# gorgonia/agogo

Measured on AMD Instinct MI355X. Metric: mcts_sims_per_sec, higher is better.
Workload: dtype f32 (Winograd F(5x5,3x3): fp32 transforms; transform-domain products as fp16x2 = each fp32 operand scaled by a power of two and split into 2 fp16 pieces (22-23 significand bits, absolute error <= 2^-38 of the tensor range), 3 fp16 MFMAs per product, fp32 accumulate)

## Files before the change

agogo_amd/csrc/conv_wino_h2.hpp:

```cpp
#pragma once

template <int TM> struct WinoT;
template <> struct WinoT<4> {
  static constexpr int AL = 6, VSHIFT = 7;
  static constexpr float BT[6][6] = {{4, 0, -5, 0, 1, 0}, {0, -4, -4, 1, 1, 0}, {0, 4, -4, -1, 1, 0}, {0, -2, -1, 2, 1, 0}, {0, 2, -1, -2, 1, 0}, {0, 4, 0, -5, 0, 1}};
  static constexpr float AT[4][6] = {{1, 1, 1, 1, 1, 0}, {0, 1, -1, 2, -2, 0}, {0, 1, 1, 4, 4, 0}, {0, 1, -1, 8, -8, 1}};
  static constexpr double G[6][3] = {{1.0 / 4, 0, 0}, {-1.0 / 6, -1.0 / 6, -1.0 / 6}, {-1.0 / 6, 1.0 / 6, -1.0 / 6}, {1.0 / 24, 1.0 / 12, 1.0 / 6}, {1.0 / 24, -1.0 / 12, 1.0 / 6}, {0, 0, 1}};
};
template <> struct WinoT<5> {
  static constexpr int AL = 7, VSHIFT = 6;
  static constexpr float BT[7][7] = {{-0.5f, 0.25f, 2.5f, -1.25f, -2, 1, 0}, {0, 0.5f, 0.25f, -2.25f, -1, 1, 0}, {0, -0.5f, 0.75f, 1.75f, -3, 1, 0},
                                     {0, 1, 1.5f, -2, -1.5f, 1, 0},          {0, -1, 2.5f, 0, -2.5f, 1, 0},       {0, 0.25f, 0, -1.25f, 0, 1, 0},
                                     {0, -0.5f, 0.25f, 2.5f, -1.25f, -2, 1}};
  static constexpr float AT[5][7] = {{1, 1, 1, 1, 1, 1, 0}, {0, 1, -1, 0.5f, -0.5f, 2, 0}, {0, 1, 1, 0.25f, 0.25f, 4, 0}, {0, 1, -1, 0.125f, -0.125f, 8, 0},
                                     {0, 1, 1, 0.0625f, 0.0625f, 16, 1}};
  static constexpr double G[7][3] = {{-2, 0, 0}, {-2.0 / 3, -2.0 / 3, -2.0 / 3}, {-2.0 / 9, 2.0 / 9, -2.0 / 9}, {16.0 / 9, 8.0 / 9, 4.0 / 9}, {16.0 / 15, -8.0 / 15, 4.0 / 15},
                                     {2.0 / 45, 4.0 / 45, 8.0 / 45}, {0, 0, 1}};
};
template <int TM> __device__ __forceinline__ void wino_btv(const float* d, float* o);
template <int TM> __device__ __forceinline__ void wino_atv(const float* m, float* o);
template <> __device__ __forceinline__ void wino_btv<4>(const float* d, float* o) { wino_bt6(d, o); }
template <> __device__ __forceinline__ void wino_atv<4>(const float* m, float* o) { wino_at4(m, o); }
template <> __device__ __forceinline__ void wino_btv<5>(const float* d, float* o) {
  o[0] = -0.5f * d[0] + 0.25f * d[1] + 2.5f * d[2] - 1.25f * d[3] - 2.f * d[4] + d[5];
// ... 33 lines not shown
  float* wave_max;
  float w_unscale;
  const float* t_in;
  const float* col_unscale;
  const float* t_next;
  int cform;
  const _Float16* U2c;
  const float* amax_true;
  const float* wm_prev;
  float* wm_out;
  unsigned* amax_next;
  float g1, g0;
  int gemm_variant;
  int temporal_stores;
  int live_r, live_c;
  int row_pad;
};
__device__ __forceinline__ size_t h2_row(const WinoH2Args& h, int pos, int t) {
  return (size_t)(t >> h.rsh) * h.rA + (size_t)pos * h.rB + (size_t)(t & h.rmask);
}

__device__ __forceinline__ void wino_h2_scales(unsigned amax_bits, int shift, float* s, float* inv) {
  int e = (int)((amax_bits >> 23) & 0xffu);
  if (amax_bits == 0u) { *s = 1.f; *inv = 1.f; return; }
  e = e < 30 ? 30 : (e > 230 ? 230 : e);
  *s = __uint_as_float((unsigned)(268 - shift - e) << 23);
  *inv = __uint_as_float((unsigned)(e - 14 + shift) << 23);
}

__device__ __forceinline__ unsigned wino_h2_pack(float a, float b, unsigned* lo) {
// ... 50 lines not shown
#pragma unroll
    for (int i = 0; i < AL; i++) {
      const bool ok = okx && TM * ty + i < a.Hp;
      dx[i] = ok ? d[i][j].x : 0.f; dy[i] = ok ? d[i][j].y : 0.f;
    }
    wino_btv<TM>(dx, ox);
    wino_btv<TM>(dy, oy);
#pragma unroll
    for (int i = 0; i < AL; i++) { tmx[i][j] = ox[i]; tmy[i][j] = oy[i]; }
  }
  unsigned* V2 = reinterpret_cast<unsigned*>(a.V);
  const int c = 2 * c2;
  const size_t word_in_row = (size_t)(c >> 5) * 32 + ((c & 31) >> 1);
  const int lane = threadIdx.x & 63;
  const size_t swap_word = (size_t)((c2 >> 6) * 4) * 32 + lane;
  const int row_r = (h.cform && h.live_r) ? maps::rows_row(maps::ROWS_R, a.nty, a.ntx, b % (128 / a.TPB), ty, tx) : (t & 127);
  const int row_c = (h.cform && h.live_c) ? maps::rows_row(maps::ROWS_C, a.nty, a.ntx, b % (128 / a.TPB), ty, tx) : (t & 127);
#pragma unroll
  for (int i = 0; i < AL; i++) {
    float ox[AL], oy[AL];
    wino_btv<TM>(tmx[i], ox);
    wino_btv<TM>(tmy[i], oy);
#pragma unroll
    for (int j = 0; j < AL; j++) {
      unsigned lo;
      const unsigned hi = wino_h2_pack(ox[j] * sbx, oy[j] * sby, &lo);
      if (h.cform) {
        const auto s16 = __builtin_amdgcn_permlane16_swap(hi, lo, false, false);
        const unsigned e0 = s16[0], e1 = s16[1];
        const int NS = a.C >> 5;
        const size_t chunk0 = ((size_t)(t >> 7) * h.npos + (size_t)(i * AL + j)) * NS + (size_t)((c2 >> 6) * 4 + 2 * (lane >> 5));
        const int cls = maps::rows_class(true, true, AL, i, j);
        const int row = cls == maps::ROWS_R ? row_r : (cls == maps::ROWS_C ? row_c : (t & 127));
        if (row < 0) continue;
        unsigned* p0 = V2 + chunk0 * 4096 + (size_t)row * 32 + (lane & 31);
        p0[0] = e0;
        p0[4096] = e1;
        continue;
      }
      unsigned* rowp = V2 + h2_row(h, i * AL + j, t) * a.C;
      if (h.in_swap) {
        const auto s16 = __builtin_amdgcn_permlane16_swap(hi, lo, false, false);
        const unsigned e0 = s16[0], e1 = s16[1];
        const auto s32 = __builtin_amdgcn_permlane32_swap(e0, e1, false, false);
        const unsigned w0 = s32[0], w1 = s32[1];
        rowp[swap_word] = w0;
        rowp[swap_word + 64] = w1;
      } else {
        rowp[word_in_row] = hi;
        rowp[word_in_row + 16] = lo;
// ... 970 lines not shown
```

agogo_amd/csrc/conv_wino_h2c.hpp:

```cpp
#pragma once

__device__ __forceinline__ unsigned h2c_img(int row, int slot) { return maps::h2c_img(row, slot); }

template <int NK, int PFA>
__global__ __launch_bounds__(256, 2) void wino_gemm_h2c_kernel(WinoH2Args h) {
  const WinoArgs& a = h.w;
  constexpr int SA = 128 * 128, SB = 256 * 128;
  __shared__ __attribute__((aligned(16))) unsigned char lds[SA + SB];

  const int n_nt = a.Ntot >> 8;
  const int per_pos = a.n_mtiles * n_nt;
  const int nblk = h.npos * per_pos;
  const int id = blockIdx.x;
  int q = nblk >> 3, rr = nblk & 7, xcd = id & 7, slot = id >> 3;
  int tile = (xcd < rr ? xcd * (q + 1) : rr * (q + 1) + (xcd - rr) * q) + slot;
  const int pos = tile / per_pos;
  const int rem = tile - pos * per_pos;
  const int m_tile = rem / n_nt, n_tile = rem - m_tile * n_nt;

  const int tid = threadIdx.x, lane = tid & 63, wid = tid >> 6;
  const int wm = wid >> 1, wn = wid & 1;
  const unsigned st_lds = h2c_img(tid >> 3, tid & 7);
  const char* abase = reinterpret_cast<const char*>(a.V) + ((size_t)m_tile * h.npos + pos) * (size_t)NK * SA + (size_t)tid * 16;
  const char* bbase = reinterpret_cast<const char*>(h.U2c) + (((size_t)pos * NK) * n_nt + n_tile) * (size_t)SB + (size_t)tid * 16;
// ... 68 lines not shown
        const unsigned w0 = s32[0], w1 = s32[1];
        float* d = mbase + (size_t)qq * 8192 + (size_t)(i * 32 + (r & 3) + 8 * (r >> 2)) * 64;
        d[0] = __uint_as_float(w0);
        d[4 * 64] = __uint_as_float(w1);
      }
}

typedef __attribute__((address_space(3))) void* h2c_lds_ptr_t;
template <int NK, bool NT = true>
__global__ __launch_bounds__(256, 3) void wino_gemm_h2g_kernel(WinoH2Args h) {
  const WinoArgs& a = h.w;
  constexpr int SA = 128 * 128, SB = 256 * 128;
  __shared__ __attribute__((aligned(16))) unsigned char lds[SA + SB];

  const int n_nt = a.Ntot >> 8;
  const int per_pos = a.n_mtiles * n_nt;
  const int nblk = h.npos * per_pos;
  const int id = blockIdx.x;
  int q = nblk >> 3, rr = nblk & 7, xcd = id & 7, slot = id >> 3;
  int tile = (xcd < rr ? xcd * (q + 1) : rr * (q + 1) + (xcd - rr) * q) + slot;
  const int pos = tile / per_pos;
  const int rem = tile - pos * per_pos;
  const int m_tile = rem / n_nt, n_tile = rem - m_tile * n_nt;

  const int tid = threadIdx.x, lane = tid & 63;
  const int wid = __builtin_amdgcn_readfirstlane(tid >> 6);
  const int wm = wid >> 1, wn = wid & 1;
  const __amdgpu_buffer_rsrc_t ar = h2_rsrc(a.V), br = h2_rsrc(h.U2c);
  const unsigned vo_e = maps::h2c_dma_src(lane, 0), vo_o = maps::h2c_dma_src(lane, 1);
  const unsigned a_w = maps::h2c_wave_part(wid, 128), b_w = maps::h2c_wave_part(wid, 256);
  unsigned a_so = (unsigned)(((size_t)m_tile * h.npos + pos) * (size_t)NK * SA) + a_w;
  unsigned b_so = (unsigned)((((size_t)pos * NK) * n_nt + n_tile) * (size_t)SB) + b_w;
  const unsigned b_step = (unsigned)n_nt * SB;
  unsigned char* const la = lds + a_w;
  unsigned char* const lb = lds + SA + b_w;

  f32x16 acc[2][4];
#pragma unroll
  for (int i = 0; i < 2; i++)
#pragma unroll
    for (int j = 0; j < 4; j++)
#pragma unroll
      for (int r = 0; r < 16; r++) acc[i][j][r] = 0.f;

  const int live = maps::rows_pos_live(h.live_r, h.live_c, h.tm + 2, pos);
  const bool a_on = maps::h2c_wave_row0(wid, 128) < live;
  const int ni = (maps::h2c_mfma_row0(wm, 0) < live ? 1 : 0) + (maps::h2c_mfma_row0(wm, 1) < live ? 1 : 0);
  auto k_loop = [&](auto ni_c) {
    constexpr int NI = decltype(ni_c)::value;
#pragma nounroll
    for (int it = 0; it < NK; it++) {
      if (a_on) {
#pragma unroll
        for (int j = 0; j < maps::h2c_wave_instrs(128); j++)
          __builtin_amdgcn_raw_ptr_buffer_load_lds(ar, (h2c_lds_ptr_t)(la + maps::h2c_dma_dst(0, j)), 16, (j & 1) ? vo_o : vo_e,
                                                   a_so + (maps::h2c_dma_src(0, j) - maps::h2c_dma_src(0, j & 1)), 0, 0);
      }
#pragma unroll
      for (int j = 0; j < maps::h2c_wave_instrs(256); j++)
        __builtin_amdgcn_raw_ptr_buffer_load_lds(br, (h2c_lds_ptr_t)(lb + maps::h2c_dma_dst(0, j)), 16, (j & 1) ? vo_o : vo_e,
                                                 b_so + (maps::h2c_dma_src(0, j) - maps::h2c_dma_src(0, j & 1)), 0, 0);
      a_so += SA; b_so += b_step;
      __syncthreads();
      if (NI > 0) {
#pragma unroll
        for (int ks = 0; ks < 2; ks++) {
          f16x8_t A_[2][2];
#pragma unroll
          for (int i = 0; i < NI; i++) {
            A_[i][0] = *reinterpret_cast<const f16x8_t*>(lds + maps::h2c_frag(maps::h2c_mfma_row0(wm, i), lane, 0, ks));
            A_[i][1] = *reinterpret_cast<const f16x8_t*>(lds + maps::h2c_frag(maps::h2c_mfma_row0(wm, i), lane, 1, ks));
          }
#pragma unroll
          for (int j = 0; j < 4; j++) {
            const f16x8_t b0 = *reinterpret_cast<const f16x8_t*>(lds + SA + maps::h2c_frag(wn * 128 + j * 32, lane, 0, ks));
            const f16x8_t b1 = *reinterpret_cast<const f16x8_t*>(lds + SA + maps::h2c_frag(wn * 128 + j * 32, lane, 1, ks));
#pragma unroll
            for (int i = 0; i < NI; i++) {
              acc[i][j] = __builtin_amdgcn_mfma_f32_32x32x16_f16(A_[i][1], b0, acc[i][j], 0, 0, 0);
              acc[i][j] = __builtin_amdgcn_mfma_f32_32x32x16_f16(A_[i][0], b1, acc[i][j], 0, 0, 0);
              acc[i][j] = __builtin_amdgcn_mfma_f32_32x32x16_f16(A_[i][0], b0, acc[i][j], 0, 0, 0);
            }
          }
        }
      }
      __syncthreads();
    }
  };
  if (ni == 2) k_loop(std::integral_constant<int, 2>{});
  else if (ni == 1) k_loop(std::integral_constant<int, 1>{});
  else k_loop(std::integral_constant<int, 0>{});

  float* mbase = a.Mb + maps::mc_index(m_tile, h.npos, pos, a.Ntot >> 6, n_tile * 4 + wn * 2, wm * 64, lane);
#pragma unroll
  for (int qq = 0; qq < 2; qq++)
#pragma unroll
    for (int i = 0; i < 2; i++) {
      if (i >= ni) continue;
#pragma unroll
      for (int r = 0; r < 16; r++) {
        const unsigned x0 = __float_as_uint(acc[i][2 * qq][r]), x1 = __float_as_uint(acc[i][2 * qq + 1][r]);
        const auto s32 = __builtin_amdgcn_permlane32_swap(x0, x1, false, false);
        const unsigned w0 = s32[0], w1 = s32[1];
        float* d = mbase + maps::mc_index(0, 0, 0, 0, qq, i * 32 + maps::mfma_row(r), 0);
        if (NT) {
          __builtin_nontemporal_store(__uint_as_float(w0), d);
          __builtin_nontemporal_store(__uint_as_float(w1), d + maps::mc_index(0, 0, 0, 0, 0, 4, 0));
        } else {
          d[0] = __uint_as_float(w0);
          d[maps::mc_index(0, 0, 0, 0, 0, 4, 0)] = __uint_as_float(w1);
        }
      }
    }
// ... 188 lines not shown
  using WT = WinoT<TM>;
  constexpr int AL = WT::AL;
  const WinoArgs& a = h.w;
  extern __shared__ __attribute__((aligned(16))) float ys[];
  const int tid = threadIdx.x, tl = tid >> 4, pr = tid & 15, lane = tid & 63;
  const int s = blockIdx.y, NS = a.C >> 5, HW = a.H * a.W;
  const int t0 = blockIdx.x * 16;
  const int t = t0 + tl;
  const bool live = t < a.T;
  const int tc = live ? t : a.T - 1;
  const int b = tc / a.TPB, tt = tc - b * a.TPB;
  const int ty = tt / a.ntx, tx = tt - ty * a.ntx;
  const int bl = tl / a.TPB;
  float s_, un0;
  wino_h2_scales(h.amax_in[b], WT::VSHIFT, &s_, &un0);
  const __amdgpu_buffer_rsrc_t mr = h2_rsrc(a.Mb + ((size_t)(t0 >> 7) * h.npos * NS + s) * 8192);
  const unsigned m_lane = (unsigned)(((tc & 127) * 64 + pr * 4) * 4);
  const unsigned m_pos = (unsigned)NS * 32768u;
  const int bpt = 128 / a.TPB;
  auto m_row = [&](int cls) -> unsigned {
    const int r = maps::rows_row(cls, a.nty, a.ntx, b % bpt, ty, tx);
    return r < 0 ? 0x80000000u : (unsigned)((r * 64 + pr * 4) * 4);
  };
  const unsigned m_lane_r = h.live_r ? m_row(maps::ROWS_R) : m_lane, m_lane_c = h.live_c ? m_row(maps::ROWS_C) : m_lane;
  auto m_voff = [&](int xi, int nu) -> unsigned {
    const int cls = maps::rows_class(true, true, AL, xi, nu);
    return cls == maps::ROWS_R ? m_lane_r : (cls == maps::ROWS_C ? m_lane_c : m_lane);
  };
  float Y[TM][TM][4];
#pragma unroll
  for (int k = 0; k < TM; k++)
#pragma unroll
    for (int l = 0; l < TM; l++)
#pragma unroll
      for (int e = 0; e < 4; e++) Y[k][l][e] = 0.f;
  float4 m[2][AL];
#pragma unroll
  for (int xi = 0; xi < AL; xi++) m[0][xi] = h2_ldf4(mr, m_voff(xi, 0), (unsigned)(xi * AL) * m_pos);
#pragma unroll
// ... 183 lines not shown
  extern __shared__ __attribute__((aligned(16))) float ys[];
  const int tid = threadIdx.x, tl = tid >> 4, pr = tid & 15, lane = tid & 63;
  const int NS = a.C >> 5;
  const int PH = TM * a.nty + 2, PW = TM * a.ntx + 2;
  const int bpg = 16 / a.TPB;
  const int n_groups = (a.T + 15) >> 4, n_items = n_groups * NS;
  const int tt = tl % a.TPB, bl = tl / a.TPB;
  const int ty = tt / a.ntx, tx = tt - ty * a.ntx;
  for (int i = tid; i < bpg * PH * PW * 32; i += 256) ys[i] = 0.f;
  const __amdgpu_buffer_rsrc_t mr = h2_rsrc(a.Mb);
  const __amdgpu_buffer_rsrc_t vr = h2_rsrc(a.V);
  const unsigned m_lane = (unsigned)((tl * 64 + pr * 4) * 4);
  const unsigned v_lane = (unsigned)((((tid >> 6) * 4) * 128) + lane * 4);
  const unsigned e_pix = (unsigned)a.Cout_p * 16u;
  constexpr unsigned OOB = 0x80000000u;
  const unsigned gr_r = h.live_r ? (unsigned)(bpg * maps::rows_per_board(maps::ROWS_R, a.nty, a.ntx)) : 16u;
  const unsigned gr_c = h.live_c ? (unsigned)(bpg * maps::rows_per_board(maps::ROWS_C, a.nty, a.ntx)) : 16u;
  auto m_row = [&](int cls) -> unsigned {
    const int r = maps::rows_row(cls, a.nty, a.ntx, bl, ty, tx);
    return r < 0 ? OOB : (unsigned)((r * 64 + pr * 4) * 4);
  };
  auto v_row = [&](int cls, int k) -> unsigned {
    const int tv = (tid >> 6) * 4 + 2 * k + (lane >> 5), ttv = tv % a.TPB;
    const int r = maps::rows_row(cls, a.nty, a.ntx, tv / a.TPB, ttv / a.ntx, ttv % a.ntx);
    return r < 0 ? OOB : (unsigned)(r * 128 + (lane & 31) * 4);
  };
  const unsigned m_lane_r = h.live_r ? m_row(maps::ROWS_R) : m_lane, m_lane_c = h.live_c ? m_row(maps::ROWS_C) : m_lane;
  const unsigned v0_r = h.live_r ? v_row(maps::ROWS_R, 0) : v_lane, v1_r = h.live_r ? v_row(maps::ROWS_R, 1) : v_lane + 256u;
  const unsigned v0_c = h.live_c ? v_row(maps::ROWS_C, 0) : v_lane, v1_c = h.live_c ? v_row(maps::ROWS_C, 1) : v_lane + 256u;
  float* const ybase = ys + ((size_t)bl * PH * PW + (size_t)(TM * ty) * PW + TM * tx) * 32 + 2 * pr;
  unsigned okmask = 0;
#pragma unroll
  for (int k = 0; k < TM; k++)
#pragma unroll
    for (int l = 0; l < TM; l++) okmask |= (TM * ty + k < a.H && TM * tx + l < a.W) ? 1u << (k * TM + l) : 0u;
  const __amdgpu_buffer_rsrc_t er = h2_rsrc(a.ep);
  float4 m[NPRE][AL];
  auto m_soff = [&](int g, int s, int xi, int nu) -> unsigned {
    const int cls = maps::rows_class(true, true, AL, xi, nu);
    const unsigned gr = cls == maps::ROWS_R ? gr_r : (cls == maps::ROWS_C ? gr_c : 16u);
    return (unsigned)((((g >> 3) * h.npos + xi * AL + nu) * NS + s)) * 32768u + (unsigned)(g & 7) * (gr * 256u);
  };
  auto m_voff = [&](int xi, int nu) -> unsigned {
    const int cls = maps::rows_class(true, true, AL, xi, nu);
    return cls == maps::ROWS_R ? m_lane_r : (cls == maps::ROWS_C ? m_lane_c : m_lane);
  };
  int item = blockIdx.x;
  {
    const int g = __builtin_amdgcn_readfirstlane(item / NS), s = __builtin_amdgcn_readfirstlane(item - (item / NS) * NS);
#pragma unroll
    for (int nu = 0; nu < NPRE; nu++)
#pragma unroll
      for (int xi = 0; xi < AL; xi++) m[nu][xi] = h2_ldf4<MAUX>(mr, m_voff(xi, nu), m_soff(g, s, xi, nu));
  }
  __syncthreads();
  for (; item < n_items; item += gridDim.x) {
    const int g = __builtin_amdgcn_readfirstlane(item / NS), s = __builtin_amdgcn_readfirstlane(item - (item / NS) * NS);
    const int t = g * 16 + tl;
    const bool live = t < a.T;
    const int b = live ? g * bpg + bl : (a.T - 1) / a.TPB;
    float s_, un0;
    wino_h2_scales(h.amax_in[b], WT::VSHIFT, &s_, &un0);
    f2c Y[TM][TM][2];
#pragma unroll
    for (int k = 0; k < TM; k++)
#pragma unroll
      for (int l = 0; l < TM; l++) { Y[k][l][0] = f2c{0.f, 0.f}; Y[k][l][1] = f2c{0.f, 0.f}; }
#pragma unroll
    for (int nu = 0; nu < AL; nu++) {
      f2c c0[AL], c1[AL], o0[TM], o1[TM];
#pragma unroll
      for (int xi = 0; xi < AL; xi++) {
        const float4 v = m[nu % NPRE][xi];
        c0[xi] = f2c{v.x, v.y}; c1[xi] = f2c{v.z, v.w};
      }
      if (nu + NPRE < AL) {
#pragma unroll
        for (int xi = 0; xi < AL; xi++) m[nu % NPRE][xi] = h2_ldf4<MAUX>(mr, m_voff(xi, nu + NPRE), m_soff(g, s, xi, nu + NPRE));
      }
      wino_atv_p<TM>(c0, o0);
      wino_atv_p<TM>(c1, o1);
#pragma unroll
      for (int k = 0; k < TM; k++) {
        f2c y0[TM], y1[TM];
#pragma unroll
        for (int l = 0; l < TM; l++) { y0[l] = Y[k][l][0]; y1[l] = Y[k][l][1]; }
        wino_at_acc_p<TM>(nu, y0, o0[k]);
        wino_at_acc_p<TM>(nu, y1, o1[k]);
#pragma unroll
        for (int l = 0; l < TM; l++) { Y[k][l][0] = y0[l]; Y[k][l][1] = y1[l]; }
      }
      __builtin_amdgcn_sched_barrier(0);
    }
// ... 45 lines not shown
      for (int o = 8; o > 0; o >>= 1) ax = fmaxf(ax, __shfl_xor(ax, o, 64));
    }
    const float bound = h.g1 * ax + h.g0;
    const unsigned bbits = __float_as_uint(bound);
    if (s == 0 && tt == 0 && pr == 0 && live) h.amax_next[b] = bbits;
    float sb, inv_;
    wino_h2_scales(bbits, WT::VSHIFT, &sb, &inv_);
    const float sv = live ? sb : 0.f;
    __syncthreads();
    {
      const int nx = item + (int)gridDim.x < n_items ? item + (int)gridDim.x : item;
      const int g2 = __builtin_amdgcn_readfirstlane(nx / NS), s2 = __builtin_amdgcn_readfirstlane(nx - (nx / NS) * NS);
#pragma unroll
      for (int nu = 0; nu < NPRE; nu++)
#pragma unroll
        for (int xi = 0; xi < AL; xi++) m[nu][xi] = h2_ldf4<MAUX>(mr, m_voff(xi, nu), m_soff(g2, s2, xi, nu));
    }
    __builtin_amdgcn_sched_barrier(0);
    const unsigned v_base = (unsigned)((((g >> 3) * h.npos) * NS + s)) * 16384u;
    const unsigned v_g = (unsigned)(g & 7) * 2048u, v_g_r = (unsigned)(g & 7) * (gr_r * 128u), v_g_c = (unsigned)(g & 7) * (gr_c * 128u);
    const unsigned v_pos = (unsigned)NS * 16384u;
    const float* yr = ybase;
    asm volatile("" : "+v"(yr));
#pragma unroll
    for (int i0 = 0; i0 < AL; i0 += 3) {
      constexpr int NRMAX = 3;
      const int nr = AL - i0 < NRMAX ? AL - i0 : NRMAX;
      f2c tmr[NRMAX][AL];
#pragma unroll
      for (int j = 0; j < AL; j++) {
        f2c d[AL];
#pragma unroll
        for (int ii = 0; ii < AL; ii++) {
          const float2 v = *reinterpret_cast<const float2*>(yr + (ii * PW + j) * 32);
          d[ii] = f2c{v.x, v.y};
        }
// ... 5 lines not shown
#pragma unroll
      for (int r = 0; r < NRMAX; r++) {
        if (r >= nr) continue;
        const int i = i0 + r;
        f2c o[AL];
        wino_btv_p<TM>(tmr[r], o);
#pragma unroll
        for (int j = 0; j < AL; j++) {
          unsigned lo;
          const unsigned hi = wino_h2_pack(o[j].x * sv, o[j].y * sv, &lo);
          const auto s16 = __builtin_amdgcn_permlane16_swap(hi, lo, false, false);
          const unsigned e0 = s16[0], e1 = s16[1];
          const auto s32 = __builtin_amdgcn_permlane32_swap(e0, e1, false, false);
          const unsigned w0 = s32[0], w1 = s32[1];
          const int cls = maps::rows_class(true, true, AL, i, j);
          const unsigned v_so = v_base + (cls == maps::ROWS_R ? v_g_r : (cls == maps::ROWS_C ? v_g_c : v_g)) + (unsigned)(i * AL + j) * v_pos;
          __builtin_amdgcn_raw_buffer_store_b32(w0, vr, cls == maps::ROWS_R ? v0_r : (cls == maps::ROWS_C ? v0_c : v_lane), v_so, VAUX);
          __builtin_amdgcn_raw_buffer_store_b32(w1, vr, cls == maps::ROWS_R ? v1_r : (cls == maps::ROWS_C ? v1_c : v_lane + 256u), v_so, VAUX);
        }
      }
      __builtin_amdgcn_sched_barrier(0);
    }
    __syncthreads();
  }
}

static void wino_build_u2c(const std::vector<_Float16>& u2, std::vector<_Float16>& u2c, int npos, int Ntot, int C, int Cout_p) {
  const int NC = C / 32, NT = Ntot / 256;
  u2c.assign(u2.size(), (_Float16)0.f);
  for (int pos = 0; pos < npos; pos++)
    for (int kc = 0; kc < NC; kc++)
      for (int nn = 0; nn < Ntot; nn++) {
        const int s = nn >> 6, j2 = nn & 63, ch = 32 * s + (j2 >> 1), br = j2 & 1, n = br * Cout_p + ch;
// ... 8 lines not shown
static inline bool wino_h2c_ok(int H, int W, int tm, int Kp) {
  const int tpb = ceil_div(H, tm) * ceil_div(W, tm);
  const int nk = Kp / 32;
  return Kp % 128 == 0 && 16 % tpb == 0 && (nk == 4 || nk == 8 || nk == 12 || nk == 16) &&
         (size_t)(16 / tpb) * (tm * ceil_div(H, tm) + 2) * (tm * ceil_div(W, tm) + 2) * 128 <= 80 * 1024;
}

static void wino_h2c_geometry(WinoH2Args& h) {
  WinoArgs& a = h.w;
  const int tm = h.tm == 5 ? 5 : 4;
  h.tm = tm; h.npos = (tm + 2) * (tm + 2);
  a.nty = ceil_div(a.H, tm); a.ntx = ceil_div(a.W, tm); a.TPB = a.nty * a.ntx; a.T = a.B * a.TPB;
  h.rsh = 7; h.rmask = 127; h.rA = (unsigned)h.npos * 128u; h.rB = 128u;
  a.n_mtiles = ceil_div(a.T, 128); a.n_ntiles = ceil_div(a.Ntot, 128);
  h.in_swap = 1; h.cform = 1; h.wm_per_board = 0;
}
constexpr int WINO_H2_GEMM_DEFAULT = 1;
static inline int wino_h2c_gemm_variant(const WinoH2Args& h) { return h.gemm_variant > 0 ? h.gemm_variant : WINO_H2_GEMM_DEFAULT; }
static inline bool wino_h2c_dma_ok(const WinoH2Args& h) {
  return wino_h2_rows(h.npos, (size_t)h.w.T) * h.w.C * 4 < ((size_t)1 << 31) && (size_t)h.npos * h.w.C * h.w.Ntot * 4 < ((size_t)1 << 31);
}
static inline bool wino_h2c_fits31(const WinoH2Args& h) { return wino_h2_rows(h.npos, (size_t)h.w.T) * h.w.Ntot * 4 < ((size_t)1 << 31); }
static bool wino_h2c_oip_ready(agz_ctx* ctx) {
  if (!(ctx->func_attr_state & 2u)) {
    const bool ok = hipFuncSetAttribute(reinterpret_cast<const void*>(&wino_oip_h2c_kernel<5>), hipFuncAttributeMaxDynamicSharedMemorySize, 80 * 1024) == hipSuccess &&
                    hipFuncSetAttribute(reinterpret_cast<const void*>(&wino_oip_h2c_kernel<4>), hipFuncAttributeMaxDynamicSharedMemorySize, 80 * 1024) == hipSuccess;
    if (!ok) (void)hipGetLastError();
    ctx->func_attr_state |= 2u | (ok ? 1u : 0u);
  }
  return (ctx->func_attr_state & 1u) != 0;
}
static void wino_h2c_rows(agz_ctx* ctx, WinoH2Args& h, int oi_variant, bool keep_all) {
  wino_h2c_geometry(h);
  h.live_r = h.live_c = 0;
  const int gemm = wino_h2c_gemm_variant(h) & 15;
  const maps::WinoRows g = maps::wino_rows(h.w.H, h.w.W, h.tm);
  if (keep_all || gemm != 1 || oi_variant != 4 || !wino_h2c_dma_ok(h) || !wino_h2c_fits31(h) || !maps::rows_short_ok(g) || !wino_h2c_oip_ready(ctx)) return;
  h.live_r = g.dead_y ? maps::rows_slot_live(g, maps::ROWS_R) : 0;
  h.live_c = g.dead_x ? maps::rows_slot_live(g, maps::ROWS_C) : 0;
}
static void wino_h2c_in(agz_ctx* ctx, WinoH2Args& h, hipStream_t st) {
  wino_h2c_geometry(h);
  h.fuse_prev = 0; h.amax_self = const_cast<unsigned*>(h.amax_in);
  ProfScopeOn ps(ctx, AGZ_PROF_WINO_IN, st == ctx->stream.raw());
  const size_t n_in = (size_t)h.w.T * (h.w.C / 2);
  if (h.tm == 5) hipLaunchKernelGGL(wino_in_h2_kernel<5>, dim3((unsigned)((n_in + 255) / 256)), dim3(256), 0, st, h);
  else hipLaunchKernelGGL(wino_in_h2_kernel<4>, dim3((unsigned)((n_in + 255) / 256)), dim3(256), 0, st, h);
}
static void wino_h2c_gemm(agz_ctx* ctx, WinoH2Args& h, hipStream_t st) {
  wino_h2c_geometry(h);
  ProfScopeOn ps(ctx, AGZ_PROF_WINO_GEMM, st == ctx->stream.raw());
  const dim3 g(h.npos * h.w.n_mtiles * (h.w.Ntot >> 8));
  const bool dma_ok = wino_h2c_dma_ok(h);
  const int variant_all = wino_h2c_gemm_variant(h);
  const int variant = variant_all & 15, mode = (variant_all >> 4) & 3;
  const int n_slabs = h.w.Ntot >> 7;
  if (variant == 2 && dma_ok && (h.w.C >> 5) == 8 && h.w.Ntot % 256 == 0 && ctx->num_cus / 8 >= n_slabs) {
    const dim3 gp((unsigned)(8 * ((ctx->num_cus / 8) / n_slabs) * n_slabs));
    switch (mode) {
      case 1: hipLaunchKernelGGL(wino_gemm_h2p_kernel<1>, gp, dim3(256), 0, st, h); break;
      case 2: hipLaunchKernelGGL(wino_gemm_h2p_kernel<2>, gp, dim3(256), 0, st, h); break;
      case 3: hipLaunchKernelGGL(wino_gemm_h2p_kernel<3>, gp, dim3(256), 0, st, h); break;
      default: hipLaunchKernelGGL(wino_gemm_h2p_kernel<0>, gp, dim3(256), 0, st, h); break;
    }
    return;
  }
  if (dma_ok && h.temporal_stores && (h.w.C >> 5) == 8) { hipLaunchKernelGGL((wino_gemm_h2g_kernel<8, false>), g, dim3(256), 0, st, h); return; }
  if (dma_ok) {
    switch (h.w.C >> 5) {
      case 4: hipLaunchKernelGGL((wino_gemm_h2g_kernel<4>), g, dim3(256), 0, st, h); return;
      case 8: hipLaunchKernelGGL((wino_gemm_h2g_kernel<8>), g, dim3(256), 0, st, h); return;
      case 12: hipLaunchKernelGGL((wino_gemm_h2g_kernel<12>), g, dim3(256), 0, st, h); return;
      default: hipLaunchKernelGGL((wino_gemm_h2g_kernel<16>), g, dim3(256), 0, st, h); return;
    }
  }
  switch (h.w.C >> 5) {
    case 4: hipLaunchKernelGGL((wino_gemm_h2c_kernel<4, 2>), g, dim3(256), 0, st, h); break;
    case 8: hipLaunchKernelGGL((wino_gemm_h2c_kernel<8, 2>), g, dim3(256), 0, st, h); break;
    case 12: hipLaunchKernelGGL((wino_gemm_h2c_kernel<12, 2>), g, dim3(256), 0, st, h); break;
    default: hipLaunchKernelGGL((wino_gemm_h2c_kernel<16, 2>), g, dim3(256), 0, st, h); break;
  }
}
static void wino_h2c_oi(agz_ctx* ctx, WinoH2Args& h, bool last, hipStream_t st, int variant = 4) {
  wino_h2c_geometry(h);
  ProfScopeOn ps(ctx, AGZ_PROF_WINO_OUT, st == ctx->stream.raw());
  const WinoArgs& a = h.w;
  const dim3 g((unsigned)ceil_div(a.T, 16), (unsigned)(a.C >> 5));
  const size_t shm = last ? 0 : (size_t)(16 / a.TPB) * a.H * a.W * 32 * sizeof(float);
// ... 23 lines not shown
```

agogo_amd/csrc/gemm_maps.hpp:

```cpp
#pragma once
#include <cstddef>
#if defined(__HIPCC__)
#define AGZ_MAPS_HD __host__ __device__
#else
#define AGZ_MAPS_HD
#endif

namespace agz {
namespace maps {

AGZ_MAPS_HD constexpr unsigned h2c_img(int row, int unit) { return (unsigned)(row * 128 + ((unit ^ ((row >> 1) & 7)) << 4)); }

AGZ_MAPS_HD constexpr unsigned h2c_dma_src(int lane, int j) {
  return (unsigned)(j * 1024 + (lane >> 3) * 128 + (((lane & 7) ^ ((4 * j + (lane >> 4)) & 7)) << 4));
}
AGZ_MAPS_HD constexpr unsigned h2c_dma_dst(int lane, int j) { return (unsigned)(j * 1024 + lane * 16); }
AGZ_MAPS_HD constexpr unsigned h2c_wave_part(int wid, int stage_rows) { return (unsigned)(wid * (stage_rows / 4) * 128); }
AGZ_MAPS_HD constexpr int h2c_wave_instrs(int stage_rows) { return stage_rows / 4 / 8; }

AGZ_MAPS_HD constexpr unsigned h2c_frag(int row0, int lane, int piece, int ks) {
  return (unsigned)((row0 + (lane & 31)) * 128 + (((piece * 4 + 2 * ks + (lane >> 5)) ^ ((lane >> 1) & 7)) << 4));
}

AGZ_MAPS_HD constexpr int mfma_row(int r) { return (r & 3) + 8 * (r >> 2); }
// ... 27 lines not shown
AGZ_MAPS_HD constexpr bool rows_live_ok(int live) { return live == 32 || live == 64 || live == 96; }
AGZ_MAPS_HD constexpr bool rows_short_ok(const WinoRows& g) {
  return 128 % g.TPB == 0 && (g.dead_y || g.dead_x) && (!g.dead_y || rows_live_ok(rows_slot_live(g, ROWS_R))) &&
         (!g.dead_x || rows_live_ok(rows_slot_live(g, ROWS_C)));
}
AGZ_MAPS_HD constexpr int rows_pos_live(int live_r, int live_c, int AL, int pos) {
  return pos / AL == AL - 1 ? (live_r ? live_r : 128) : ((live_c && pos % AL == AL - 1) ? live_c : 128);
}
AGZ_MAPS_HD constexpr int rows_stored_per_board(const WinoRows& g) {
  int n = 0;
  for (int xi = 0; xi < g.AL; xi++)
    for (int nu = 0; nu < g.AL; nu++) n += rows_per_board(rows_class(g.dead_y, g.dead_x, g.AL, xi, nu), g.nty, g.ntx);
  return n;
}

constexpr int H2P_D = 10, H2P_R = 16, H2P_NK = 8;
AGZ_MAPS_HD constexpr unsigned h2p_v_base(int pos, int hm, int npos) {
  return (unsigned)(((hm >> 1) * npos + pos) * (H2P_NK * 16384) + (hm & 1) * 8192);
}
AGZ_MAPS_HD constexpr int h2p_slot(int par, int kk) { return (par * H2P_NK + kk) % H2P_R; }
AGZ_MAPS_HD constexpr int h2p_slot_next(int par, int kk) { return (par * H2P_NK + kk + 1) % H2P_R; }
AGZ_MAPS_HD constexpr int h2p_slot_ahead(int par, int kk) { return (par * H2P_NK + kk + H2P_D) % H2P_R; }
AGZ_MAPS_HD constexpr int h2p_kk_ahead(int kk) { return (kk + H2P_D) % H2P_NK; }
AGZ_MAPS_HD constexpr int h2p_tiles_ahead(int kk) { return (kk + H2P_D) / H2P_NK; }
AGZ_MAPS_HD constexpr int h2p_wait_steady() { return 4 + (H2P_D - 2) * 6; }
AGZ_MAPS_HD constexpr int h2p_wait_early() { return (H2P_D - 2) * 2; }
AGZ_MAPS_HD constexpr bool h2p_early(int t) { return t < 2; }
struct H2pTeam { int team, slab, nteams; bool idle; };
AGZ_MAPS_HD constexpr H2pTeam h2p_team(int block, int grid, int n_slabs) {
  const int xcd = block & 7, slot = block >> 3, tpx = (grid >> 3) / n_slabs;
// ... 7 lines not shown
```

Measured before the change: 44520.

## Pack dead-row Winograd positions densely across slots and shrink GEMM grid

Positions whose tile rows are partly dead (the last row or column of the transform grid) now pack live rows from several 128-row slots into shared slots. The GEMM launch only covers the tiles actually used, instead of running every tile and masking inactive waves. The input transform, GEMM tile mapping and output transform are all updated with the new packed slot and row addressing. This drops the per-tile live-row specialisation in the GEMM for a simpler uniform loop, but the address arithmetic becomes more complex and the producer and consumer layouts must stay consistent.

```diff
diff --git a/agogo_amd/csrc/conv_wino_h2.hpp b/agogo_amd/csrc/conv_wino_h2.hpp
--- a/agogo_amd/csrc/conv_wino_h2.hpp
+++ b/agogo_amd/csrc/conv_wino_h2.hpp
@@ -71,6 +71,7 @@
   int gemm_variant;
   int temporal_stores;
   int live_r, live_c;
+  maps::PackGrid pk;
   int row_pad;
 };
 __device__ __forceinline__ size_t h2_row(const WinoH2Args& h, int pos, int t) {
@@ -151,8 +152,12 @@
   const size_t word_in_row = (size_t)(c >> 5) * 32 + ((c & 31) >> 1);
   const int lane = threadIdx.x & 63;
   const size_t swap_word = (size_t)((c2 >> 6) * 4) * 32 + lane;
-  const int row_r = (h.cform && h.live_r) ? maps::rows_row(maps::ROWS_R, a.nty, a.ntx, b % (128 / a.TPB), ty, tx) : (t & 127);
-  const int row_c = (h.cform && h.live_c) ? maps::rows_row(maps::ROWS_C, a.nty, a.ntx, b % (128 / a.TPB), ty, tx) : (t & 127);
+  auto packed = [&](int cls, int S) -> int {
+    const int idx = maps::rows_row(cls, a.nty, a.ntx, 0, ty, tx);
+    return idx < 0 ? -1 : maps::pack_slot_row(S, 128 / a.TPB, maps::rows_per_board(cls, a.nty, a.ntx), b, idx);
+  };
+  const int row_r = (h.cform && h.live_r) ? packed(maps::ROWS_R, h.pk.S_r) : t;
+  const int row_c = (h.cform && h.live_c) ? packed(maps::ROWS_C, h.pk.S_c) : t;
 #pragma unroll
   for (int i = 0; i < AL; i++) {
     float ox[AL], oy[AL];
@@ -166,11 +171,11 @@
         const auto s16 = __builtin_amdgcn_permlane16_swap(hi, lo, false, false);
         const unsigned e0 = s16[0], e1 = s16[1];
         const int NS = a.C >> 5;
-        const size_t chunk0 = ((size_t)(t >> 7) * h.npos + (size_t)(i * AL + j)) * NS + (size_t)((c2 >> 6) * 4 + 2 * (lane >> 5));
         const int cls = maps::rows_class(true, true, AL, i, j);
-        const int row = cls == maps::ROWS_R ? row_r : (cls == maps::ROWS_C ? row_c : (t & 127));
+        const int row = cls == maps::ROWS_R ? row_r : (cls == maps::ROWS_C ? row_c : t);
         if (row < 0) continue;
-        unsigned* p0 = V2 + chunk0 * 4096 + (size_t)row * 32 + (lane & 31);
+        const size_t chunk0 = ((size_t)(row >> 7) * h.npos + (size_t)(i * AL + j)) * NS + (size_t)((c2 >> 6) * 4 + 2 * (lane >> 5));
+        unsigned* p0 = V2 + chunk0 * 4096 + (size_t)(row & 127) * 32 + (lane & 31);
         p0[0] = e0;
         p0[4096] = e1;
         continue;
diff --git a/agogo_amd/csrc/conv_wino_h2c.hpp b/agogo_amd/csrc/conv_wino_h2c.hpp
--- a/agogo_amd/csrc/conv_wino_h2c.hpp
+++ b/agogo_amd/csrc/conv_wino_h2c.hpp
@@ -106,14 +106,11 @@
   __shared__ __attribute__((aligned(16))) unsigned char lds[SA + SB];
 
   const int n_nt = a.Ntot >> 8;
-  const int per_pos = a.n_mtiles * n_nt;
-  const int nblk = h.npos * per_pos;
+  const int nblk = maps::pack_grid_tiles(h.pk);
   const int id = blockIdx.x;
   int q = nblk >> 3, rr = nblk & 7, xcd = id & 7, slot = id >> 3;
-  int tile = (xcd < rr ? xcd * (q + 1) : rr * (q + 1) + (xcd - rr) * q) + slot;
-  const int pos = tile / per_pos;
-  const int rem = tile - pos * per_pos;
-  const int m_tile = rem / n_nt, n_tile = rem - m_tile * n_nt;
+  const maps::PackTile pt = maps::pack_tile(h.pk, (xcd < rr ? xcd * (q + 1) : rr * (q + 1) + (xcd - rr) * q) + slot);
+  const int pos = pt.pos, m_tile = pt.slot, n_tile = pt.n_tile;
 
   const int tid = threadIdx.x, lane = tid & 63;
   const int wid = __builtin_amdgcn_readfirstlane(tid >> 6);
@@ -135,60 +132,46 @@
 #pragma unroll
       for (int r = 0; r < 16; r++) acc[i][j][r] = 0.f;
 
-  const int live = maps::rows_pos_live(h.live_r, h.live_c, h.tm + 2, pos);
-  const bool a_on = maps::h2c_wave_row0(wid, 128) < live;
-  const int ni = (maps::h2c_mfma_row0(wm, 0) < live ? 1 : 0) + (maps::h2c_mfma_row0(wm, 1) < live ? 1 : 0);
-  auto k_loop = [&](auto ni_c) {
-    constexpr int NI = decltype(ni_c)::value;
 #pragma nounroll
-    for (int it = 0; it < NK; it++) {
-      if (a_on) {
-#pragma unroll
-        for (int j = 0; j < maps::h2c_wave_instrs(128); j++)
-          __builtin_amdgcn_raw_ptr_buffer_load_lds(ar, (h2c_lds_ptr_t)(la + maps::h2c_dma_dst(0, j)), 16, (j & 1) ? vo_o : vo_e,
-                                                   a_so + (maps::h2c_dma_src(0, j) - maps::h2c_dma_src(0, j & 1)), 0, 0);
-      }
-#pragma unroll
-      for (int j = 0; j < maps::h2c_wave_instrs(256); j++)
-        __builtin_amdgcn_raw_ptr_buffer_load_lds(br, (h2c_lds_ptr_t)(lb + maps::h2c_dma_dst(0, j)), 16, (j & 1) ? vo_o : vo_e,
-                                                 b_so + (maps::h2c_dma_src(0, j) - maps::h2c_dma_src(0, j & 1)), 0, 0);
-      a_so += SA; b_so += b_step;
-      __syncthreads();
-      if (NI > 0) {
-#pragma unroll
-        for (int ks = 0; ks < 2; ks++) {
-          f16x8_t A_[2][2];
-#pragma unroll
-          for (int i = 0; i < NI; i++) {
-            A_[i][0] = *reinterpret_cast<const f16x8_t*>(lds + maps::h2c_frag(maps::h2c_mfma_row0(wm, i), lane, 0, ks));
-            A_[i][1] = *reinterpret_cast<const f16x8_t*>(lds + maps::h2c_frag(maps::h2c_mfma_row0(wm, i), lane, 1, ks));
-          }
-#pragma unroll
-          for (int j = 0; j < 4; j++) {
-            const f16x8_t b0 = *reinterpret_cast<const f16x8_t*>(lds + SA + maps::h2c_frag(wn * 128 + j * 32, lane, 0, ks));
-            const f16x8_t b1 = *reinterpret_cast<const f16x8_t*>(lds + SA + maps::h2c_frag(wn * 128 + j * 32, lane, 1, ks));
-#pragma unroll
-            for (int i = 0; i < NI; i++) {
-              acc[i][j] = __builtin_amdgcn_mfma_f32_32x32x16_f16(A_[i][1], b0, acc[i][j], 0, 0, 0);
-              acc[i][j] = __builtin_amdgcn_mfma_f32_32x32x16_f16(A_[i][0], b1, acc[i][j], 0, 0, 0);
-              acc[i][j] = __builtin_amdgcn_mfma_f32_32x32x16_f16(A_[i][0], b0, acc[i][j], 0, 0, 0);
-            }
-          }
+  for (int it = 0; it < NK; it++) {
+#pragma unroll
+    for (int j = 0; j < maps::h2c_wave_instrs(128); j++)
+      __builtin_amdgcn_raw_ptr_buffer_load_lds(ar, (h2c_lds_ptr_t)(la + maps::h2c_dma_dst(0, j)), 16, (j & 1) ? vo_o : vo_e,
+                                               a_so + (maps::h2c_dma_src(0, j) - maps::h2c_dma_src(0, j & 1)), 0, 0);
+#pragma unroll
+    for (int j = 0; j < maps::h2c_wave_instrs(256); j++)
+      __builtin_amdgcn_raw_ptr_buffer_load_lds(br, (h2c_lds_ptr_t)(lb + maps::h2c_dma_dst(0, j)), 16, (j & 1) ? vo_o : vo_e,
+                                               b_so + (maps::h2c_dma_src(0, j) - maps::h2c_dma_src(0, j & 1)), 0, 0);
+    a_so += SA; b_so += b_step;
+    __syncthreads();
+#pragma unroll
+    for (int ks = 0; ks < 2; ks++) {
+      f16x8_t A_[2][2];
+#pragma unroll
+      for (int i = 0; i < 2; i++) {
+        A_[i][0] = *reinterpret_cast<const f16x8_t*>(lds + maps::h2c_frag(maps::h2c_mfma_row0(wm, i), lane, 0, ks));
+        A_[i][1] = *reinterpret_cast<const f16x8_t*>(lds + maps::h2c_frag(maps::h2c_mfma_row0(wm, i), lane, 1, ks));
+      }
+#pragma unroll
+      for (int j = 0; j < 4; j++) {
+        const f16x8_t b0 = *reinterpret_cast<const f16x8_t*>(lds + SA + maps::h2c_frag(wn * 128 + j * 32, lane, 0, ks));
+        const f16x8_t b1 = *reinterpret_cast<const f16x8_t*>(lds + SA + maps::h2c_frag(wn * 128 + j * 32, lane, 1, ks));
+#pragma unroll
+        for (int i = 0; i < 2; i++) {
+          acc[i][j] = __builtin_amdgcn_mfma_f32_32x32x16_f16(A_[i][1], b0, acc[i][j], 0, 0, 0);
+          acc[i][j] = __builtin_amdgcn_mfma_f32_32x32x16_f16(A_[i][0], b1, acc[i][j], 0, 0, 0);
+          acc[i][j] = __builtin_amdgcn_mfma_f32_32x32x16_f16(A_[i][0], b0, acc[i][j], 0, 0, 0);
         }
       }
-      __syncthreads();
-    }
-  };
-  if (ni == 2) k_loop(std::integral_constant<int, 2>{});
-  else if (ni == 1) k_loop(std::integral_constant<int, 1>{});
-  else k_loop(std::integral_constant<int, 0>{});
+    }
+    __syncthreads();
+  }
 
   float* mbase = a.Mb + maps::mc_index(m_tile, h.npos, pos, a.Ntot >> 6, n_tile * 4 + wn * 2, wm * 64, lane);
 #pragma unroll
   for (int qq = 0; qq < 2; qq++)
 #pragma unroll
     for (int i = 0; i < 2; i++) {
-      if (i >= ni) continue;
 #pragma unroll
       for (int r = 0; r < 16; r++) {
         const unsigned x0 = __float_as_uint(acc[i][2 * qq][r]), x1 = __float_as_uint(acc[i][2 * qq + 1][r]);
@@ -407,15 +390,19 @@
   const int bl = tl / a.TPB;
   float s_, un0;
   wino_h2_scales(h.amax_in[b], WT::VSHIFT, &s_, &un0);
-  const __amdgpu_buffer_rsrc_t mr = h2_rsrc(a.Mb + ((size_t)(t0 >> 7) * h.npos * NS + s) * 8192);
-  const unsigned m_lane = (unsigned)(((tc & 127) * 64 + pr * 4) * 4);
+  const int sl0 = (t0 >> 7) & ~3;
+  const __amdgpu_buffer_rsrc_t mr = h2_rsrc(a.Mb + ((size_t)sl0 * h.npos * NS + s) * 8192);
   const unsigned m_pos = (unsigned)NS * 32768u;
+  const unsigned m_slot = (unsigned)h.npos * m_pos;
+  const unsigned m_lane = (unsigned)((t0 >> 7) - sl0) * m_slot + (unsigned)(((tc & 127) * 64 + pr * 4) * 4);
   const int bpt = 128 / a.TPB;
-  auto m_row = [&](int cls) -> unsigned {
-    const int r = maps::rows_row(cls, a.nty, a.ntx, b % bpt, ty, tx);
-    return r < 0 ? 0x80000000u : (unsigned)((r * 64 + pr * 4) * 4);
-  };
-  const unsigned m_lane_r = h.live_r ? m_row(maps::ROWS_R) : m_lane, m_lane_c = h.live_c ? m_row(maps::ROWS_C) : m_lane;
+  auto m_row = [&](int cls, int S) -> unsigned {
+    const int idx = maps::rows_row(cls, a.nty, a.ntx, 0, ty, tx);
+    if (idx < 0) return 0x80000000u;
+    const int p = maps::pack_slot_row(S, bpt, maps::rows_per_board(cls, a.nty, a.ntx), b, idx);
+    return (unsigned)((p >> 7) - sl0) * m_slot + (unsigned)(((p & 127) * 64 + pr * 4) * 4);
+  };
+  const unsigned m_lane_r = h.live_r ? m_row(maps::ROWS_R, h.pk.S_r) : m_lane, m_lane_c = h.live_c ? m_row(maps::ROWS_C, h.pk.S_c) : m_lane;
   auto m_voff = [&](int xi, int nu) -> unsigned {
     const int cls = maps::rows_class(true, true, AL, xi, nu);
     return cls == maps::ROWS_R ? m_lane_r : (cls == maps::ROWS_C ? m_lane_c : m_lane);
@@ -629,6 +616,8 @@
   const unsigned v_lane = (unsigned)((((tid >> 6) * 4) * 128) + lane * 4);
   const unsigned e_pix = (unsigned)a.Cout_p * 16u;
   constexpr unsigned OOB = 0x80000000u;
+  const int S_r = h.pk.S_r, S_c = h.pk.S_c;
+  const unsigned m_dq = (unsigned)(h.npos * NS - 1) * 32768u, v_dq = (unsigned)(h.npos * NS - 1) * 16384u;
   const unsigned gr_r = h.live_r ? (unsigned)(bpg * maps::rows_per_board(maps::ROWS_R, a.nty, a.ntx)) : 16u;
   const unsigned gr_c = h.live_c ? (unsigned)(bpg * maps::rows_per_board(maps::ROWS_C, a.nty, a.ntx)) : 16u;
   auto m_row = [&](int cls) -> unsigned {
@@ -654,11 +643,14 @@
   auto m_soff = [&](int g, int s, int xi, int nu) -> unsigned {
     const int cls = maps::rows_class(true, true, AL, xi, nu);
     const unsigned gr = cls == maps::ROWS_R ? gr_r : (cls == maps::ROWS_C ? gr_c : 16u);
-    return (unsigned)((((g >> 3) * h.npos + xi * AL + nu) * NS + s)) * 32768u + (unsigned)(g & 7) * (gr * 256u);
-  };
-  auto m_voff = [&](int xi, int nu) -> unsigned {
+    const int S = cls == maps::ROWS_R ? S_r : (cls == maps::ROWS_C ? S_c : 1);
+    return (unsigned)(((maps::pack_group_slot0(S, g) * h.npos + xi * AL + nu) * NS + s)) * 32768u + maps::pack_group_rg0(S, g, gr) * 256u;
+  };
+  auto m_voff = [&](int g, int xi, int nu) -> unsigned {
     const int cls = maps::rows_class(true, true, AL, xi, nu);
-    return cls == maps::ROWS_R ? m_lane_r : (cls == maps::ROWS_C ? m_lane_c : m_lane);
+    if (cls == maps::ROWS_R) return m_lane_r + maps::pack_q(S_r, maps::pack_group_rg0(S_r, g, gr_r), m_lane_r, 8) * m_dq;
+    if (cls == maps::ROWS_C) return m_lane_c + maps::pack_q(S_c, maps::pack_group_rg0(S_c, g, gr_c), m_lane_c, 8) * m_dq;
+    return m_lane;
   };
   int item = blockIdx.x;
   {
@@ -666,7 +658,7 @@
 #pragma unroll
     for (int nu = 0; nu < NPRE; nu++)
 #pragma unroll
-      for (int xi = 0; xi < AL; xi++) m[nu][xi] = h2_ldf4<MAUX>(mr, m_voff(xi, nu), m_soff(g, s, xi, nu));
+      for (int xi = 0; xi < AL; xi++) m[nu][xi] = h2_ldf4<MAUX>(mr, m_voff(g, xi, nu), m_soff(g, s, xi, nu));
   }
   __syncthreads();
   for (; item < n_items; item += gridDim.x) {
@@ -691,7 +683,7 @@
       }
       if (nu + NPRE < AL) {
 #pragma unroll
-        for (int xi = 0; xi < AL; xi++) m[nu % NPRE][xi] = h2_ldf4<MAUX>(mr, m_voff(xi, nu + NPRE), m_soff(g, s, xi, nu + NPRE));
+        for (int xi = 0; xi < AL; xi++) m[nu % NPRE][xi] = h2_ldf4<MAUX>(mr, m_voff(g, xi, nu + NPRE), m_soff(g, s, xi, nu + NPRE));
       }
       wino_atv_p<TM>(c0, o0);
       wino_atv_p<TM>(c1, o1);
@@ -767,12 +759,20 @@
 #pragma unroll
       for (int nu = 0; nu < NPRE; nu++)
 #pragma unroll
-        for (int xi = 0; xi < AL; xi++) m[nu][xi] = h2_ldf4<MAUX>(mr, m_voff(xi, nu), m_soff(g2, s2, xi, nu));
+        for (int xi = 0; xi < AL; xi++) m[nu][xi] = h2_ldf4<MAUX>(mr, m_voff(g2, xi, nu), m_soff(g2, s2, xi, nu));
     }
     __builtin_amdgcn_sched_barrier(0);
-    const unsigned v_base = (unsigned)((((g >> 3) * h.npos) * NS + s)) * 16384u;
-    const unsigned v_g = (unsigned)(g & 7) * 2048u, v_g_r = (unsigned)(g & 7) * (gr_r * 128u), v_g_c = (unsigned)(g & 7) * (gr_c * 128u);
     const unsigned v_pos = (unsigned)NS * 16384u;
+    const unsigned v_slot = (unsigned)h.npos * v_pos;
+    const unsigned rg0_r = maps::pack_group_rg0(S_r, g, gr_r), rg0_c = maps::pack_group_rg0(S_c, g, gr_c);
+    const unsigned v_g = (unsigned)(g >> 3) * v_slot + (unsigned)s * 16384u + (unsigned)(g & 7) * 2048u;
+    const unsigned v_g_r = maps::pack_group_slot0(S_r, g) * v_slot + (unsigned)s * 16384u + rg0_r * 128u;
+    const unsigned v_g_c = maps::pack_group_slot0(S_c, g) * v_slot + (unsigned)s * 16384u + rg0_c * 128u;
+    auto v_voff = [&](int cls, int k) -> unsigned {
+      if (cls == maps::ROWS_R) { const unsigned o = k ? v1_r : v0_r; return o + maps::pack_q(S_r, rg0_r, o, 7) * v_dq; }
+      if (cls == maps::ROWS_C) { const unsigned o = k ? v1_c : v0_c; return o + maps::pack_q(S_c, rg0_c, o, 7) * v_dq; }
+      return k ? v_lane + 256u : v_lane;
+    };
     const float* yr = ybase;
     asm volatile("" : "+v"(yr));
 #pragma unroll
@@ -808,9 +808,9 @@
           const auto s32 = __builtin_amdgcn_permlane32_swap(e0, e1, false, false);
           const unsigned w0 = s32[0], w1 = s32[1];
           const int cls = maps::rows_class(true, true, AL, i, j);
-          const unsigned v_so = v_base + (cls == maps::ROWS_R ? v_g_r : (cls == maps::ROWS_C ? v_g_c : v_g)) + (unsigned)(i * AL + j) * v_pos;
-          __builtin_amdgcn_raw_buffer_store_b32(w0, vr, cls == maps::ROWS_R ? v0_r : (cls == maps::ROWS_C ? v0_c : v_lane), v_so, VAUX);
-          __builtin_amdgcn_raw_buffer_store_b32(w1, vr, cls == maps::ROWS_R ? v1_r : (cls == maps::ROWS_C ? v1_c : v_lane + 256u), v_so, VAUX);
+          const unsigned v_so = (cls == maps::ROWS_R ? v_g_r : (cls == maps::ROWS_C ? v_g_c : v_g)) + (unsigned)(i * AL + j) * v_pos;
+          __builtin_amdgcn_raw_buffer_store_b32(w0, vr, v_voff(cls, 0), v_so, VAUX);
+          __builtin_amdgcn_raw_buffer_store_b32(w1, vr, v_voff(cls, 1), v_so, VAUX);
         }
       }
       __builtin_amdgcn_sched_barrier(0);
@@ -849,6 +849,12 @@
   h.rsh = 7; h.rmask = 127; h.rA = (unsigned)h.npos * 128u; h.rB = 128u;
   a.n_mtiles = ceil_div(a.T, 128); a.n_ntiles = ceil_div(a.Ntot, 128);
   h.in_swap = 1; h.cform = 1; h.wm_per_board = 0;
+  h.pk = maps::pack_grid(tm + 2, a.nty, a.ntx, a.B, a.Ntot >> 8, h.live_r, h.live_c);
+}
+static int wino_h2c_gemm_tiles(const WinoH2Args& h) {
+  int n = 0;
+  for (int pos = 0; pos < h.npos; pos++) n += maps::pack_pos_used(h.pk, pos);
+  return n * h.pk.n_nt;
 }
 constexpr int WINO_H2_GEMM_DEFAULT = 1;
 static inline int wino_h2c_gemm_variant(const WinoH2Args& h) { return h.gemm_variant > 0 ? h.gemm_variant : WINO_H2_GEMM_DEFAULT; }
@@ -873,6 +879,7 @@
   if (keep_all || gemm != 1 || oi_variant != 4 || !wino_h2c_dma_ok(h) || !wino_h2c_fits31(h) || !maps::rows_short_ok(g) || !wino_h2c_oip_ready(ctx)) return;
   h.live_r = g.dead_y ? maps::rows_slot_live(g, maps::ROWS_R) : 0;
   h.live_c = g.dead_x ? maps::rows_slot_live(g, maps::ROWS_C) : 0;
+  wino_h2c_geometry(h);
 }
 static void wino_h2c_in(agz_ctx* ctx, WinoH2Args& h, hipStream_t st) {
   wino_h2c_geometry(h);
@@ -900,13 +907,14 @@
     }
     return;
   }
-  if (dma_ok && h.temporal_stores && (h.w.C >> 5) == 8) { hipLaunchKernelGGL((wino_gemm_h2g_kernel<8, false>), g, dim3(256), 0, st, h); return; }
+  const dim3 gd((unsigned)wino_h2c_gemm_tiles(h));
+  if (dma_ok && h.temporal_stores && (h.w.C >> 5) == 8) { hipLaunchKernelGGL((wino_gemm_h2g_kernel<8, false>), gd, dim3(256), 0, st, h); return; }
   if (dma_ok) {
     switch (h.w.C >> 5) {
-      case 4: hipLaunchKernelGGL((wino_gemm_h2g_kernel<4>), g, dim3(256), 0, st, h); return;
-      case 8: hipLaunchKernelGGL((wino_gemm_h2g_kernel<8>), g, dim3(256), 0, st, h); return;
-      case 12: hipLaunchKernelGGL((wino_gemm_h2g_kernel<12>), g, dim3(256), 0, st, h); return;
-      default: hipLaunchKernelGGL((wino_gemm_h2g_kernel<16>), g, dim3(256), 0, st, h); return;
+      case 4: hipLaunchKernelGGL((wino_gemm_h2g_kernel<4>), gd, dim3(256), 0, st, h); return;
+      case 8: hipLaunchKernelGGL((wino_gemm_h2g_kernel<8>), gd, dim3(256), 0, st, h); return;
+      case 12: hipLaunchKernelGGL((wino_gemm_h2g_kernel<12>), gd, dim3(256), 0, st, h); return;
+      default: hipLaunchKernelGGL((wino_gemm_h2g_kernel<16>), gd, dim3(256), 0, st, h); return;
     }
   }
   switch (h.w.C >> 5) {
diff --git a/agogo_amd/csrc/gemm_maps.hpp b/agogo_amd/csrc/gemm_maps.hpp
--- a/agogo_amd/csrc/gemm_maps.hpp
+++ b/agogo_amd/csrc/gemm_maps.hpp
@@ -65,6 +65,42 @@
   return n;
 }
 
+AGZ_MAPS_HD constexpr int pack_slots(int live) { return live == 96 || live == 32 ? 4 : (live == 64 ? 2 : 1); }
+AGZ_MAPS_HD constexpr int pack_used_per_group(int live) { return live == 96 ? 3 : 1; }
+AGZ_MAPS_HD constexpr int pack_rg(int S, int bpt, int l, int b, int idx) { return (b % (S * bpt)) * l + idx; }
+AGZ_MAPS_HD constexpr int pack_slot_row(int S, int bpt, int l, int b, int idx) { return (b / (S * bpt)) * S * 128 + pack_rg(S, bpt, l, b, idx); }
+AGZ_MAPS_HD constexpr int pack_used_slots(int S, int bpt, int l, int B) {
+  return (B / (S * bpt)) * (S * bpt * l / 128) + ((B % (S * bpt)) * l + 127) / 128;
+}
+AGZ_MAPS_HD constexpr unsigned pack_group_rg0(int S, int g, int gr) { return (unsigned)((g & (8 * S - 1)) * gr); }
+AGZ_MAPS_HD constexpr int pack_log2(int S) { return S >> 1; }
+AGZ_MAPS_HD constexpr unsigned pack_group_slot0(int S, int g) { return (unsigned)((g >> (3 + pack_log2(S))) << pack_log2(S)); }
+AGZ_MAPS_HD constexpr unsigned pack_q(int S, unsigned rg0, unsigned off, int row_shift) { return ((rg0 + (off >> row_shift)) >> 7) & (unsigned)(S - 1); }
+struct PackGrid { int AL, n_nt, u_full, u_r, u_c, S_r, S_c, per_r, per_c; };
+AGZ_MAPS_HD constexpr PackGrid pack_grid(int AL, int nty, int ntx, int B, int n_nt, int live_r, int live_c) {
+  const int TPB = nty * ntx, bpt = 128 / TPB, u_full = pack_used_slots(1, bpt, TPB, B);
+  return PackGrid{AL, n_nt, u_full,
+                  live_r ? pack_used_slots(pack_slots(live_r), bpt, rows_per_board(ROWS_R, nty, ntx), B) : u_full,
+                  live_c ? pack_used_slots(pack_slots(live_c), bpt, rows_per_board(ROWS_C, nty, ntx), B) : u_full,
+                  pack_slots(live_r), pack_slots(live_c), pack_used_per_group(live_r), pack_used_per_group(live_c)};
+}
+AGZ_MAPS_HD constexpr int pack_pos_used(const PackGrid& g, int pos) {
+  return pos / g.AL == g.AL - 1 ? g.u_r : (pos % g.AL == g.AL - 1 ? g.u_c : g.u_full);
+}
+AGZ_MAPS_HD constexpr int pack_grid_tiles(const PackGrid& g) {
+  return ((g.AL - 1) * ((g.AL - 1) * g.u_full + g.u_c) + g.AL * g.u_r) * g.n_nt;
+}
+struct PackTile { int pos, slot, n_tile; };
+AGZ_MAPS_HD constexpr PackTile pack_tile(const PackGrid& g, int tile) {
+  const int u = tile / g.n_nt, row_u = (g.AL - 1) * g.u_full + g.u_c;
+  const int xi = u / row_u < g.AL - 1 ? u / row_u : g.AL - 1, r = u - xi * row_u;
+  const bool last = xi == g.AL - 1;
+  const int nu = last ? r / g.u_r : (r / g.u_full < g.AL - 1 ? r / g.u_full : g.AL - 1);
+  const int k = r - nu * (last ? g.u_r : g.u_full);
+  const int per = last ? g.per_r : (nu == g.AL - 1 ? g.per_c : 1), S = last ? g.S_r : (nu == g.AL - 1 ? g.S_c : 1);
+  return PackTile{xi * g.AL + nu, (k / per) * S + k % per, tile - u * g.n_nt};
+}
+
 constexpr int H2P_D = 10, H2P_R = 16, H2P_NK = 8;
 AGZ_MAPS_HD constexpr unsigned h2p_v_base(int pos, int hm, int npos) {
   return (unsigned)(((hm >> 1) * npos + pos) * (H2P_NK * 16384) + (hm & 1) * 8192);
```

Result: faster. 45440, median of 6 (+2.1%).
